# hello-robot/stretch_mujoco

Hardware: AMD Instinct MI355X
Metric: env-steps/sec (whole node), 4096 parallel Stretch envs in total (higher is better)
Workload: dtype f32

## Files before the change

stretch_mujoco_amd/csrc/smj_builds.h:

```cpp
#pragma once
#define SMJ_BUILDS_INCLUDED 1

#define SMJ_BUILDS(X) \
  X(step) X(pgs) X(prof) X(tall) X(mid) X(midp) X(big38) X(big38p) X(big50) X(big50p) X(big) X(sat) X(sat1) X(sat2) X(satp) X(sat32) X(sat32n)
#define SMJ_CARRIES_NEWTON 1
#define SMJ_CARRIES_PGS 2
#define SMJ_CARRIES_BOTH 3
#define SMJ_FAM_STD 0
#define SMJ_FAM_TALL 1
#define SMJ_FAM_MID 2
#define SMJ_FAM_BIG38 3
#define SMJ_FAM_BIG50 4
#define SMJ_FAM_BIG 5
#define SMJ_FAM_SAT16 6
#define SMJ_FAM_SAT32 7
#define SMJ_ROW_step    SMJ_FAM_STD,   SMJ_CARRIES_NEWTON, SMJ_CARRIES_NEWTON, 1, 0, 0
#define SMJ_ROW_pgs     SMJ_FAM_STD,   SMJ_CARRIES_PGS,    SMJ_CARRIES_PGS,    1, 0, 0
#define SMJ_ROW_prof    SMJ_FAM_STD,   SMJ_CARRIES_BOTH,   SMJ_CARRIES_BOTH,   1, 0, 1
#define SMJ_ROW_tall    SMJ_FAM_TALL,  SMJ_CARRIES_BOTH,   SMJ_CARRIES_BOTH,   1, 1, 0
#define SMJ_ROW_mid     SMJ_FAM_MID,   SMJ_CARRIES_NEWTON, SMJ_CARRIES_BOTH,   1, 0, 0
#define SMJ_ROW_midp    SMJ_FAM_MID,   SMJ_CARRIES_PGS,    SMJ_CARRIES_PGS,    1, 0, 0
#define SMJ_ROW_big38   SMJ_FAM_BIG38, SMJ_CARRIES_NEWTON, SMJ_CARRIES_BOTH,   1, 0, 0
#define SMJ_ROW_big38p  SMJ_FAM_BIG38, SMJ_CARRIES_PGS,    SMJ_CARRIES_PGS,    1, 0, 0
#define SMJ_ROW_big50   SMJ_FAM_BIG50, SMJ_CARRIES_NEWTON, SMJ_CARRIES_BOTH,   1, 0, 0
#define SMJ_ROW_big50p  SMJ_FAM_BIG50, SMJ_CARRIES_PGS,    SMJ_CARRIES_PGS,    1, 0, 0
#define SMJ_ROW_big     SMJ_FAM_BIG,   SMJ_CARRIES_BOTH,   SMJ_CARRIES_BOTH,   1, 1, 0
#define SMJ_ROW_sat     SMJ_FAM_SAT16, SMJ_CARRIES_NEWTON, SMJ_CARRIES_NEWTON, 1, 0, 0
#define SMJ_ROW_sat1    SMJ_FAM_SAT16, SMJ_CARRIES_PGS,    SMJ_CARRIES_PGS,    1, 0, 0
#define SMJ_ROW_sat2    SMJ_FAM_SAT16, SMJ_CARRIES_NEWTON, SMJ_CARRIES_NEWTON, 2, 0, 0
#define SMJ_ROW_satp    SMJ_FAM_SAT16, SMJ_CARRIES_PGS,    SMJ_CARRIES_PGS,    2, 0, 0
#define SMJ_ROW_sat32   SMJ_FAM_SAT32, SMJ_CARRIES_BOTH,   SMJ_CARRIES_BOTH,   1, 1, 0
#define SMJ_ROW_sat32n  SMJ_FAM_SAT32, SMJ_CARRIES_NEWTON, SMJ_CARRIES_NEWTON, 2, 1, 0
#define SMJ_LEAN_BUILDS(X) X(lean)
#define SMJ_ROW_lean    SMJ_FAM_STD,   SMJ_CARRIES_NEWTON, SMJ_CARRIES_NEWTON, 1, 0, 0
#define smj_step_kernel_step smj_step_kernel
#define smj_launch_step_step smj_launch_step

#define SMJ_CAT2(a, b) a##b
#define SMJ_CAT(a, b) SMJ_CAT2(a, b)
#define SMJ_STR2(a) #a
#define SMJ_STR(a) SMJ_STR2(a)
#define SMJ_COLUMN(m, ...) m(__VA_ARGS__, ~)
#define SMJ_COL0(a, ...) a
#define SMJ_COL1(a, b, ...) b
#define SMJ_COL2(a, b, c, ...) c
#define SMJ_COL3(a, b, c, d, ...) d
#define SMJ_COL4(a, b, c, d, e, ...) e
#define SMJ_COL5(a, b, c, d, e, f, ...) f
#ifdef SMJ_BUILD_TAG
// ... 94 lines not shown
  SmjLaunch launch;
  bool carries(int solver) const { return (solvers & (solver == 2 ? SMJ_CARRIES_NEWTON : SMJ_CARRIES_PGS)) != 0; }
};
#define SMJ_BUILD_DESC_INIT(launcher)                                                                                          \
  {SMJ_STR(SMJ_BUILD_TAG), SMJ_BUILD_FAMILY, SMJ_STR(SMJ_STEP_KERNEL), SMJ_BUILD_WORKER_NAME, {NVP, NBP, NENT, NEFC, NCON, NVS, NSAT}, \
   SMJ_DEBUG_FLOATS, SMJ_SOLVERS, SMJ_BUILD_WAVES, SMJ_PROFILING, launcher}
enum SmjBuildId {
#define X(tag) SMJ_B_##tag,
  SMJ_BUILDS(X)
#undef X
  SMJ_B_COUNT
};
#define X(tag) extern const SmjBuildDesc smj_build_##tag;
SMJ_BUILDS(X)
SMJ_LEAN_BUILDS(X)
#undef X
```

stretch_mujoco_amd/csrc/smj_capi.hip:

```cpp
#include <hip/hip_runtime.h>
#include <dlfcn.h>
#include <rccl/rccl.h>
#include <stdarg.h>
#include <sys/stat.h>
#include <time.h>
#include <unistd.h>
#include <stdio.h>
#include <stdlib.h>
#include <string.h>

#include <initializer_list>
#include <string>
#include <vector>

#include "../../include/smj.h"
#include "../../include/smj_build.h"
#include "smj_kernels.h"
#include "smj_step_plan.h"
#include "smj_model_load.h"
#include "smj_bvh.h"
#include "smj_meshlet.h"
#include "smj_render.h"
#include "smj_points.h"
#include "smj_hmap.h"
// ... 546 lines not shown
  StagePlan in, out;
  const SmjStageLayout& Y = c->layout;
  in.add(st.qpos, m.nq_all, Y.qpos); in.add(st.qvel, m.nv_all, Y.qvel); in.add(st.warm, m.nv_all, Y.warm);
  in.add(st.ctrl, m.nu, Y.ctrl); in.add(st.bctl, SMJ_BC_ROWS, Y.bctl); in.add(st.nstep, 1, Y.nstep);
  in.add(st.info, 4, Y.info);
  out = in;
  out.add(st.act_len, m.nu, Y.actlen); out.add(st.act_vel, m.nu, Y.actvel); out.add(st.base, 3, Y.base);
  if (read_flags & SMJ_READ_IMU) { out.add(st.gyro, 3, Y.gyro); out.add(st.accel, 3, Y.accel); }
  if (read_flags & SMJ_READ_POSES) out.add(st.xpose, 12 * m.nbody_all, Y.xpose);
  st.stage = c->stage;
  st.lay = Y;
  st.cost = c->cost;
  const SmjVariant& V = smj_variants[c->variant];
  const SmjCallFacts facts{c->num_envs, nsteps, st.debug != nullptr, st.prof != nullptr, c->has_esc};
  const SmjRoute route = smj_route_lean(smj_route(c->variant, c->model.solver, facts.prof_bound, c->opt.newton_two_waves, c->opt.pgs_two_waves, smj_builds),
                                        smj_lean_facts(c->model, st, c->opt.lean_build), smj_builds[SMJ_B_step], &smj_build_lean);
  const SmjStepPlan plan = smj_plan_step(V, route, c->opt, facts);
  c->last_primary = route.primary;
  if (plan.esc) {
#define X(name, field, type) c->model_esc.field = c->model.field;
    SMJ_SOLVER_OPTIONS(X)
#undef X
  }
  hipStream_t sm = (hipStream_t)stream;
  smj_launch_stage(in, c->stage, Y.stride, c->num_envs, st.ld, false, sm);
  st.progress = st.done_steps = st.sched = st.hot = nullptr;
  if (plan.clear_sched) {
    st.progress = c->progress;
    st.done_steps = c->progress + c->num_envs;
    st.sched = c->progress + 2 * (size_t)c->num_envs;
    st.hot = st.sched + SMJ_SCHED_WORDS;
// ... 394 lines not shown
```

stretch_mujoco_amd/csrc/smj_step_impl.h:

```cpp
#pragma once
#ifndef SMJ_PROFILING
#define SMJ_PROFILING 1
#endif
#include <cstddef>
#include "smj_model.h"
#include "smj_wave.h"
#include "smj_sat_mem.h"

#define JS (NVS + 1)
#define MS (NVS + 1)
#define SMJ_MINVAL 1e-15f
#define SMJ_MINIMP 0.0001f
#define SMJ_MAXIMP 0.9999f

enum { JT_FREE = 0, JT_BALL = 1, JT_SLIDE = 2, JT_HINGE = 3 };
enum { GT_PLANE = 0, GT_SPHERE = 2, GT_CAPSULE = 3, GT_ELLIPSOID = 4, GT_CYLINDER = 5, GT_BOX = 6, GT_MESH = 7 };
enum { CT_EQUALITY = 0, CT_FRICTION = 1, CT_LIMIT = 3, CT_CONTACT_FRICTIONLESS = 5, CT_CONTACT_ELLIPTIC = 7, CT_NONE = -1 };

#if NSAT > 0
#define NCGS (NCG + 1)
#define NSURV 128
#else
#define NCGS NCG
#endif
#if defined(SMJ_TWO_WAVES) && defined(SMJ_ONLY_NEWTON) && NSAT > 0 && !defined(SMJ_EMUL)
#define SMJ_SPLIT_COLLIDE 1
#else
#define SMJ_SPLIT_COLLIDE 0
#endif
#ifndef SMJ_W2_FORWARD
#define SMJ_W2_FORWARD SMJ_SPLIT_COLLIDE
#endif
#ifndef SMJ_W2_NEWTON
#define SMJ_W2_NEWTON SMJ_SPLIT_COLLIDE
#endif
#ifndef SMJ_W2_INTEGRATE
#define SMJ_W2_INTEGRATE SMJ_SPLIT_COLLIDE
#endif
struct TreeTmp {
  float cinert[NBP][10], crb[NBP][10], cvel[NBP][6], cfrc[NBP][6], buf[NVP][6], cdof[NVP][6], cdof_dot[NVP][6];
};

#define NEFP 64
#if NSAT > 0
#define NEFC_P SMJ_SAT_PGS
#else
#define NEFC_P (NEFC > 160 ? 160 : NEFC)
#endif
#define NPS ((NEFC_P + 63) / 64)
struct Smem {
  float MM[NVS][MS];
  float Mdiag[NVP], Dinv[NVP];
  float xpos[NBT][3], xquat[NBT][4], xmat[NBT][9], com[NBT][3];
  float xaxis[NVP][3], xanchor[NVP][3];
  float qpos[NVP + 8], qvel[NVP], ctrl[16], g[NVP], uu[NVP], w[NVP], qacc[NVP], warm[NVP], tmp[NVP];
  float act_force[16], act_len[16], act_vel[16], act_free[16];
  float bctl[SMJ_BC_ROWS];
  int etype[NEFC], eid[NEFC];
  int estate[NEFC];
  float epos[NEFC], emargin[NEFC], ediag[NEFC], efloss[NEFC], eR[NEFC], eK[NEFC], eBv[NEFC], eimp[NEFC], earef[NEFC],
      eb[NEFC], ef[NEFC];
  float cpos[NCON][3], cframe[NCON][9], cdist[NCON], cfric[NCON][5], csolref[NCON][2], csolimp[NCON][5], cmargin[NCON];
#if NSAT > 0
  int cdim[NCON], cefc[NCON];
  unsigned short cgeom1[NCON], cgeom2[NCON];
  int cpair[NCON];
#else
  int cdim[NCON], cgeom1[NCON], cgeom2[NCON], cefc[NCON];
#endif
#if NSAT > 0
  float J[NDR + 1][JS];
#else
  float J[NEFC][JS];
#endif
  union {
    TreeTmp t;
    struct {
      float pos[NCGS][3], mat[NCGS][9], cen[NCGS][3], half[NCGS][3];
      float ccen[NCGS][3], size[NCGS][3];
      int meta[NCGS];
      unsigned short list[1024];
// ... 28 lines not shown
#else
      union {
        float H[NVS][NVS + 1];
        float cH[NCON][36];
      };
#endif
      int rxi[3][NEFC > 64 ? NEFC - 64 : 1];
      float rxf[15][NEFC > 64 ? NEFC - 64 : 1];
    } n;
  } u;
#if NSAT > 0
  SatMem sat;
#endif
#if SMJ_SPLIT_COLLIDE
  int mbox[4];
#endif
  SMJ_DEV float* A(int cap) { return &J[cap][0]; }
};
#define ROWPASS(rb, ne) _Pragma("unroll") for (int rb = 0; rb < NEFC; rb += 64) if (rb == 0 || __builtin_expect((ne) > rb, 0))
#define ROWPASS_ALL(rb) _Pragma("unroll") for (int rb = 0; rb < NEFC; rb += 64)
#if NEFC > 128
#define ROWS_BEGIN_(rb, ne, LOAD) _Pragma("unroll") for (int rp_ = 0; rp_ < 2; rp_++) _Pragma("nounroll") for (int rb = rp_ ? 64 : 0; rp_ ? (rb < NEFC && (ne) > rb) : rb < 64; rb += 64) { NRow nrx_; if (rp_ && (LOAD)) rx_load(nrx_, rb); NRow& nr = rp_ ? nrx_ : nr0; (void)nr;
#define ROWS_END_RW(rb) if (rp_) rx_store(nrx_, rb); }
#else
#define ROWS_BEGIN_(rb, ne, LOAD) ROWPASS(rb, ne) { NRow nrx_; if (rb != 0 && (LOAD)) rx_load(nrx_, rb); NRow& nr = (rb != 0) ? nrx_ : nr0; (void)nr;
#define ROWS_END_RW(rb) if (rb != 0) rx_store(nrx_, rb); }
#endif
#define ROWS_BEGIN(rb, ne) ROWS_BEGIN_(rb, ne, true)
#define ROWS_END_RO() }
static inline int smj_pgs_rows_static() {
  const size_t a_sq = offsetof(Smem, J) + sizeof(float) * (NEFP * JS + NEFP * NEFP);
  if (a_sq > sizeof(Smem)) return 0;
  for (int n = NEFC_P & ~15; n > NEFP; n -= 16)
// ... 544 lines not shown
      }
    }
    SYNC();
    LANES {
      const int b = lane;
      if (b > 0 && b < nb) {
        const float* R = s.xmat[b];
        const float* I = bt.inl[lane];
        float Il[9] = {I[0], I[3], I[4], I[3], I[1], I[5], I[4], I[5], I[2]}, RI[9], T[9], Rt[9];
        mulmat3(RI, R, Il);
        for (int i = 0; i < 3; i++)
          for (int j = 0; j < 3; j++) Rt[3 * i + j] = R[3 * j + i];
        mulmat3(T, RI, Rt);
        float dif[3] = {xip[lane][0] - s.com[b][0], xip[lane][1] - s.com[b][1], xip[lane][2] - s.com[b][2]};
        const float mass = I[9], dd = dot3(dif, dif);
        float* c = s.u.t.cinert[b];
        c[0] = T[0] + mass * (dd - dif[0] * dif[0]); c[1] = T[4] + mass * (dd - dif[1] * dif[1]);
        c[2] = T[8] + mass * (dd - dif[2] * dif[2]); c[3] = T[1] - mass * dif[0] * dif[1];
        c[4] = T[2] - mass * dif[0] * dif[2]; c[5] = T[5] - mass * dif[1] * dif[2];
        c[6] = mass * dif[0]; c[7] = mass * dif[1]; c[8] = mass * dif[2]; c[9] = mass;
      }
      if (lane < nv) {
        const int d = lane, b = dt.body[lane];
        float off[3] = {s.com[b][0] - s.xanchor[d][0], s.com[b][1] - s.xanchor[d][1], s.com[b][2] - s.xanchor[d][2]};
        float* c = cdof[lane];
        const int jt = dt.jtype[lane], k = d - dt.first[lane];
        if (jt == JT_SLIDE || (jt == JT_FREE && k < 3)) {
          c[0] = c[1] = c[2] = 0;
          for (int x = 0; x < 3; x++) c[3 + x] = s.xaxis[d][x];
        } else {
          for (int x = 0; x < 3; x++) c[x] = s.xaxis[d][x];
          cross3(c + 3, s.xaxis[d], off);
        }
        for (int x = 0; x < 6; x++) s.u.t.cdof[d][x] = c[x];
        qvel_r[lane] = s.qvel[d];
      } else {
        for (int x = 0; x < 6; x++) cdof[lane][x] = 0;
        qvel_r[lane] = 0;
      }
    }
    SYNC();
    LANES {
      if (lane < nv)
        for (int x = 0; x < 6; x++) s.u.t.buf[lane][x] = cdof[lane][x] * qvel_r[lane];
    }
    SYNC();
    PL<float[6]> cvb;
    LANES {
      float sv[6] = {0, 0, 0, 0, 0, 0};
      if (lane > 0 && lane < nb) {
        const int da = bt.dofadr[lane], dn = bt.dofnum[lane];
#pragma unroll
        for (int u = 0; u < 6; u++) {
          const float on = u < dn ? 1.f : 0.f;
          const int a = da + (u < dn ? u : 0);
          for (int x = 0; x < 6; x++) sv[x] += on * s.u.t.buf[dn > 0 ? a : 0][x];
        }
      }
      for (int x = 0; x < 6; x++) { cvb[lane][x] = sv[x]; if (lane < NBP) s.u.t.cvel[lane][x] = sv[x]; }
    }
    SYNC();
#pragma unroll
    for (int r = 0; r < 6; r++) {
      if (r >= M.njump) break;
      PL<float[6]> up;
      PL<int> anc;
      LANES {
        const int a = bt.jump[lane][r];
        anc[lane] = a;
        for (int x = 0; x < 6; x++) up[lane][x] = s.u.t.cvel[a][x];
      }
      SYNC();
      LANES {
        if (anc[lane] > 0)
          for (int x = 0; x < 6; x++) { cvb[lane][x] += up[lane][x]; s.u.t.cvel[lane][x] = cvb[lane][x]; }
      }
      SYNC();
    }
    LANES {
      if (lane < nv) {
        const int b = dt.body[lane], pb = M.body_parentid[b], da = M.body_dofadr[b];
        float cv[6];
        for (int x = 0; x < 6; x++) cv[x] = s.u.t.cvel[pb][x];
        const uint64_t mk = dt.velmask[lane];
#pragma unroll
        for (int u = 0; u < 5; u++) {
          const int a = da + u;
          const float on = (a < lane && ((mk >> a) & 1)) ? 1.f : 0.f;
          for (int x = 0; x < 6; x++) cv[x] += on * s.u.t.buf[a < lane ? a : lane][x];
        }
        const int jt = dt.jtype[lane], k = lane - dt.first[lane];
        if (jt == JT_FREE && k < 3) { for (int x = 0; x < 6; x++) cdof_dot[lane][x] = 0; }
        else cross_motion(cdof_dot[lane], cv, cdof[lane]);
        for (int x = 0; x < 6; x++) s.u.t.cdof_dot[lane][x] = cdof_dot[lane][x];
      } else {
        for (int x = 0; x < 6; x++) cdof_dot[lane][x] = 0;
      }
    }
    {
      PL<float[10]> cr;
      LANES { for (int k = 0; k < 10; k++) cr[lane][k] = 0.f; }
      for (int x0 = 0; x0 < M.maxsubtree; x0 += 4) {
        LANES {
          if (lane > 0 && lane < nb) {
            const int sub = bt.subsize[lane];
#pragma unroll
            for (int u = 0; u < 4; u++) {
              const bool in = x0 + u < sub;
              const int x = lane + (in ? x0 + u : 0);
              const float on = in ? 1.f : 0.f;
              for (int k = 0; k < 10; k++) cr[lane][k] += on * s.u.t.cinert[x][k];
            }
          }
        }
      }
      LANES {
        if (lane < nb)
          for (int k = 0; k < 10; k++) s.u.t.crb[lane][k] = cr[lane][k];
      }
    }
    SYNC();
    LANES {
      if (lane < nv) {
        float bf[6];
        mul_inert_vec(bf, s.u.t.crb[dt.body[lane]], cdof[lane]);
        for (int x = 0; x < 6; x++) s.u.t.buf[lane][x] = bf[x];
      }
    }
    SYNC();
    LANES {
      for (int t = 0; t < NENT; t++) {
        const int i = et.i[lane][t], j = et.j[lane][t];
        if (i < 0) continue;
        float v = 0;
        for (int x = 0; x < 6; x++) v += s.u.t.cdof[j][x] * s.u.t.buf[i][x];
        if (i == j) { v += et.arm[lane][t]; s.Mdiag[i] = v; }
        s.MM[i][j] = v;
        if (i != j) s.MM[j][i] = v;
      }
    }
    SYNC();
  }

  SMJ_DEV void factor() {
    const int nv = M.nv;
    EntryTab et;
    load(et, false);
    for (int k = nv - 1; k >= 0; k--) {
      const float dkk = s.MM[k][k], dinv = 1.0f / dkk;
      LANES {
// ... 42 lines not shown
    BodyTab bt;
    load(bt);
    LANES {
      if (lane < 16) {
        float off[3] = {0, 0, 0}, F[3] = {0, 0, 0};
        int mlo = 0, mhi = 0;
        if (lane < M.ngc) {
          const int b = at.gc_body[lane];
          const float gm = at.gc_mass[lane];
          const float lp[3] = {at.gc_x[lane], at.gc_y[lane], at.gc_z[lane]};
          float pt[3];
          mulmat3vec(pt, s.xmat[b], lp);
          for (int k = 0; k < 3; k++) { off[k] = pt[k] + s.xpos[b][k] - s.com[b][k]; F[k] = -M.gravity[k] * gm; }
          mlo = at.gc_mlo[lane]; mhi = at.gc_mhi[lane];
        }
        float* o = s.u.t.buf[lane];
        for (int k = 0; k < 3; k++) { o[k] = off[k]; o[3 + k] = F[k]; }
        s.u.t.cfrc[lane][0] = __builtin_bit_cast(float, mlo); s.u.t.cfrc[lane][1] = __builtin_bit_cast(float, mhi);
      }
    }
    SYNC();
    LANES {
      if (lane < nv) {
        float acc = 0;
#pragma unroll
        for (int t = 0; t < 16; t++) {
          const uint64_t mk = mk64(__builtin_bit_cast(int, s.u.t.cfrc[t][0]), __builtin_bit_cast(int, s.u.t.cfrc[t][1]));
          const float* o = s.u.t.buf[t];
          float tv[3];
          cross3(tv, cdof[lane], o);
          const float v = (cdof[lane][3] + tv[0]) * o[3] + (cdof[lane][4] + tv[1]) * o[4] + (cdof[lane][5] + tv[2]) * o[5];
          acc += ((mk >> lane) & 1) ? v : 0.f;
        }
        frc_passive[lane] += acc;
      }
    }
    SYNC();
    LANES {
      if (lane < nv)
        for (int x = 0; x < 6; x++) s.u.t.buf[lane][x] = s.u.t.cdof_dot[lane][x] * s.qvel[lane];
    }
    SYNC();
    PL<float[6]> ca;
    LANES {
      float sv[6] = {0, 0, 0, 0, 0, 0};
      if (lane > 0 && lane < nb) {
        const int da = bt.dofadr[lane], dn = bt.dofnum[lane];
#pragma unroll
        for (int u = 0; u < 6; u++) {
          const float on = u < dn ? 1.f : 0.f;
          const int a = dn > 0 ? da + (u < dn ? u : 0) : 0;
          for (int x = 0; x < 6; x++) sv[x] += on * s.u.t.buf[a][x];
        }
      }
      for (int x = 0; x < 6; x++) { ca[lane][x] = sv[x]; if (lane < NBP) s.u.t.cfrc[lane][x] = sv[x]; }
    }
    SYNC();
#pragma unroll
    for (int r = 0; r < 6; r++) {
      if (r >= M.njump) break;
      PL<float[6]> up;
      PL<int> anc;
      LANES {
        const int a = bt.jump[lane][r];
        anc[lane] = a;
        for (int x = 0; x < 6; x++) up[lane][x] = s.u.t.cfrc[a][x];
      }
      SYNC();
      LANES {
        if (anc[lane] > 0)
          for (int x = 0; x < 6; x++) { ca[lane][x] += up[lane][x]; s.u.t.cfrc[lane][x] = ca[lane][x]; }
      }
      SYNC();
    }
    LANES {
      if (lane < nb) {
        const int b = lane;
        float t1[6] = {0, 0, 0, 0, 0, 0}, cf[6] = {0, 0, 0, 0, 0, 0};
        if (b > 0) {
          const float a[6] = {ca[lane][0], ca[lane][1], ca[lane][2], ca[lane][3] - M.gravity[0], ca[lane][4] - M.gravity[1], ca[lane][5] - M.gravity[2]};
          float t2[6];
          mul_inert_vec(t1, s.u.t.cinert[b], a);
          mul_inert_vec(t2, s.u.t.cinert[b], s.u.t.cvel[b]);
          cross_force(cf, s.u.t.cvel[b], t2);
        }
        for (int x = 0; x < 6; x++) s.u.t.cfrc[b][x] = t1[x] + cf[x];
      }
    }
    SYNC();
    {
      PL<float[6]> cfs;
      LANES { for (int k = 0; k < 6; k++) cfs[lane][k] = 0.f; }
      for (int x0 = 0; x0 < M.maxsubtree; x0 += 4) {
        LANES {
          if (lane < nv) {
            const int b = dt.body[lane], sub = dt.bsub[lane];
#pragma unroll
            for (int u = 0; u < 4; u++) {
              const bool in = x0 + u < sub;
              const int x = b + (in ? x0 + u : 0);
              const float on = in ? 1.f : 0.f;
              for (int k = 0; k < 6; k++) cfs[lane][k] += on * s.u.t.cfrc[x][k];
            }
          }
        }
      }
      LANES {
        float v = 0;
        if (lane < nv)
          for (int k = 0; k < 6; k++) v += cdof[lane][k] * cfs[lane][k];
        frc_bias[lane] = v;
      }
    }
    LANES {
      if (lane < nu) {
        const int a = lane;
        float len = 0, vel = 0;
// ... 1710 lines not shown
      while (mask) {
        const int l = ffs64(mask);
        mask &= mask - 1;
        const int t = wave_read(tt, l);
        const int* r = static_cast<const int*>(__builtin_assume_aligned(M.k_cprec + t * SMJ_CP_STRIDE, 16));
        const float sd[3] = {wave_read(sdx, l), wave_read(sdy, l), wave_read(sdz, l)};
        narrow_pair(r, uni(r[SMJ_CP_S1]), uni(r[SMJ_CP_S2]), sepbase ? sepbase + 4 * (t & (SMJ_SEP_SLOTS / 2 - 1)) : nullptr, t + 1,
                    sepbase && wave_read(stag, l) == t + 1, sd, pc, prof);
      }
      CTICK(SMJ_PROF_C_NARROW)
    }
    SYNC();
#undef CTICK
  }

  SMJ_DEV void make_constraint() {
    const int nv = M.nv, neq = M.neq, nfric = M.nfric, nlimit = M.nlimit;
    ROWPASS(rb, nefc) LANES {
      const int row = lane + rb;
      static_assert((64 * JS) % 4 == 0 && ((NEFC % 64) * JS) % 4 == 0, "row blocks are whole float4s");
      const int nrow = NEFC - rb < 64 ? NEFC - rb : 64, nf4 = nrow * JS / 4;
      Vec4* jz = reinterpret_cast<Vec4*>(&s.J[rb][0]);
      for (int k = lane; k < nf4; k += 64) jz[k] = Vec4{0.f, 0.f, 0.f, 0.f};
      if (row < NEFC) {
        s.etype[row] = CT_NONE; s.efloss[row] = 0; s.eid[row] = 0; s.epos[row] = 0; s.emargin[row] = 0; s.ediag[row] = 0;
      }
    }
    SYNC();
    int cap = newton() ? NEFC : M.pgs_cap > 0 ? M.pgs_cap : NEFC_P;
    if (M.row_limit > 0 && M.row_limit < cap) cap = M.row_limit;
// ... 44 lines not shown
    LANES {
      if (act[lane]) {
        const int r = row0 + popc64(lm & ((1ull << lane) - 1));
        if (r < cap) {
          const int side = lrow[1][lane];
          s.J[r][lrow[0][lane]] = (float)(-side);
          s.etype[r] = CT_LIMIT; s.eid[r] = lane;
          s.epos[r] = side * (asf(lrow[2][lane]) - lq[lane]);
          s.emargin[r] = asf(lrow[3][lane]); s.ediag[r] = asf(lrow[4][lane]);
        }
      }
    }
    row0 += popc64(lm);
    if (row0 > cap) { row0 = cap; flags |= SMJ_FLAG_EFC_OVERFLOW; }
    SYNC();
    PL<int> cact, cdimv, crow;
    PL<float> ctran, crot;
    LANES {
      int act = 0, dim = 0;
      float tran = 0, rot = 0;
      if (lane < ncon) {
        const int c = lane;
        dim = s.cdim[c];
        act = s.cdist[c] < s.cmargin[c];
        const int g1 = s.cgeom1[c], g2 = s.cgeom2[c], b1 = M.geom_bodyid[g1], b2 = M.geom_bodyid[g2];
        s.u.k.b1[c] = b1; s.u.k.b2[c] = b2;
        s.u.k.m1lo[c] = M.k_body_dofmask_lo[b1]; s.u.k.m1hi[c] = M.k_body_dofmask_hi[b1];
        s.u.k.m2lo[c] = M.k_body_dofmask_lo[b2]; s.u.k.m2hi[c] = M.k_body_dofmask_hi[b2];
        tran = M.geom_invweight0[2 * g1] + M.geom_invweight0[2 * g2];
        rot = M.geom_invweight0[2 * g1 + 1] + M.geom_invweight0[2 * g2 + 1];
// ... 1497 lines not shown
    sat_integrate(bad);
#endif
    if (wave_ballot(bad) != 0) {
      flags |= SMJ_FLAG_BAD_STATE;
      LANES {
        for (int k = lane; k < M.nq; k += 64) s.qpos[k] = M.qpos0[k];
        if (lane < nv) { s.qvel[lane] = 0.f; s.warm[lane] = 0.f; }
      }
#if NSAT > 0
      sat_reset_state();
#endif
      SYNC();
    }
  }

  SMJ_DEV void imu() {
    if (M.imu_site < 0 || (!S.gyro && !staged())) return;
    const int sid = M.imu_site, b = M.site_bodyid[sid];
    const uint64_t mk = mk64(M.k_body_dofmask_lo[b], M.k_body_dofmask_hi[b]);
    float cv[6], ca[6];
    for (int x = 0; x < 6; x++) {
      PL<float> tv, ta;
      LANES {
        const bool in = (mk >> lane) & 1;
        tv[lane] = in ? cdof[lane][x] * qvel_r[lane] : 0.f;
        ta[lane] = in ? cdof_dot[lane][x] * qvel_r[lane] + cdof[lane][x] * qacc_r[lane] : 0.f;
      }
      cv[x] = wave_sum(tv); ca[x] = wave_sum(ta);
    }
    for (int k = 0; k < 3; k++) ca[3 + k] -= M.gravity[k];
// ... 6 lines not shown
    cross3(t, cv, off);
    for (int k = 0; k < 3; k++) vlin[k] = cv[3 + k] + t[k];
    cross3(t, ca, off);
    for (int k = 0; k < 3; k++) alin[k] = ca[3 + k] + t[k];
    cross3(c2, cv, vlin);
    for (int k = 0; k < 3; k++) alin[k] += c2[k];
    mulmat3Tvec(gy, R, cv);
    mulmat3Tvec(ac, R, alin);
    if (staged()) {
      float* st = stage_row();
      LANES { if (lane < 3) { st[S.lay.gyro + lane] = gy[lane]; st[S.lay.accel + lane] = ac[lane]; } }
    } else {
      LANES { if (lane < 3) { S.gyro[lane * S.ld + env] = gy[lane]; S.accel[lane * S.ld + env] = ac[lane]; } }
    }
  }

  SMJ_DEV void dump_poses() {
    if (staged()) {
      float* st = stage_row() + S.lay.xpose;
      LANES {
        for (int k = lane; k < 12 * (M.nbody + M.nsat); k += 64) {
          const int b = k / 12, c = k - 12 * b;
          st[k] = c < 3 ? s.xpos[b][c] : s.xmat[b][c - 3];
        }
      }
      return;
    }
    if (!S.xpose) return;
    LANES {
      if (lane < M.nbody + M.nsat) {
// ... 82 lines not shown
#endif
  SMJ_DEV void run(int nsteps, unsigned read_flags) {
    const int want_imu = read_flags & 1;
    flags = 0; nefc = NEFC; ncon = 0; niter = 0;
    float pc[SMJ_PROF_SLOTS];
    for (int k = 0; k < SMJ_PROF_SLOTS; k++) pc[k] = 0.f;
    const bool prof = SMJ_PROFILING && S.prof != nullptr;
    const long long tlaunch = S.cost ? smj_clock() : 0;
    long long t0 = prof ? smj_clock() : 0, tstart = t0;
#define TICK(slot) if (prof) { const long long t1 = smj_clock(); pc[slot] += (float)(t1 - t0); t0 = t1; }
    setup();
    load_state();
    TICK(SMJ_PROF_SETUP)
    for (int st = 0; st < nsteps; st++) {
      const bool last = st == nsteps - 1;
#if SMJ_W2_FORWARD
      fork2(W2_SAT_FORWARD, env);
      kinematics();
      WG_BARRIER();
#else
      kinematics();
#if NSAT > 0
      sat_forward();
#endif
#endif
      if (last && (read_flags & 4)) dump_poses();
      TICK(SMJ_PROF_KIN)
      com_crb();
      if (last) dump_debug();
      TICK(SMJ_PROF_COMCRB)
// ... 17 lines not shown
          SYNC();
          ncon = ncon_planes;
          flags = flags_planes;
          serial_redo = true;
        }
        serial_redo = false;
      }
      if (last) dump_contacts();
      TICK(SMJ_PROF_COLLISION)
#if NSAT > 0
      make_constraint_sat(pc, prof);
#else
      if (!newton()) nefc = NEFC;
      make_constraint();
#endif
      TICK(SMJ_PROF_MAKECON)
      if (S.redo && !S.redo_worker && (flags & (SMJ_FLAG_EFC_OVERFLOW | SMJ_FLAG_CON_OVERFLOW))) {
        escalate(st);
        if (S.cost) { const int cst = (int)((smj_clock() - tlaunch) >> 6); LANES { if (lane == 0) st_coh(&S.cost[env], step_base ? ld_coh(&S.cost[env]) + cst : cst); } }
        return;
      }
#if NSAT > 0
      if (newton()) solve_newton(last, pc, t0, prof);
      else solve_pgs_sat(last, pc, t0, prof);
      if (last && debug_bound()) {
        LANES {
          if (lane >= 32 && lane - 32 < M.nsat)
            for (int k = 0; k < 6; k++) S.debug[(SMJ_DBG_SATQACC + 6 * (lane - 32) + k) * S.ld + env] = s.sat.x[SX_QA][lane - 32][k];
        }
      }
// ... 26 lines not shown
```

stretch_mujoco_amd/csrc/smj_step_tu.h:

```cpp
#pragma once
#ifdef SMJ_BUILDS_INCLUDED
#error "smj_step_tu.h must be the first include of its translation unit: smj_builds.h has to see SMJ_STEP_TU"
#endif
#define SMJ_STEP_TU 1
#include "smj_builds.h"
#include "smj_step_plan.h"
#include "smj_kernels.h"
#include "smj_step_impl.h"

#define SMJ_ALOAD(p) __hip_atomic_load((p), __ATOMIC_RELAXED, __HIP_MEMORY_SCOPE_AGENT)
#define SMJ_ASTORE(p, v) __hip_atomic_store((p), (v), __ATOMIC_RELAXED, __HIP_MEMORY_SCOPE_AGENT)
#define SMJ_WAIT_TICKS 300000000LL

struct SmjTicket { int env, steps, chunk; unsigned read_flags; bool go; };
static __device__ __forceinline__ SmjTicket smj_take_ticket(const DevState& S, int nsteps, unsigned read_flags) {
  SmjTicket t;
  int slot = blockIdx.x;
  t.chunk = 0; t.steps = nsteps; t.read_flags = read_flags; t.go = true; t.env = 0;
  if (S.pipe_len) {
    t.chunk = (int)blockIdx.x / S.B;
    slot = (int)blockIdx.x - t.chunk * S.B;
    const int base = t.chunk * S.pipe_len;
    t.steps = nsteps - base < S.pipe_len ? nsteps - base : S.pipe_len;
    if (base + t.steps < nsteps) t.read_flags = 0;
// ... 12 lines not shown
        break;
      }
      if (late) {
        if (threadIdx.x == 0) atomicOr(&reinterpret_cast<int*>(S.stage + (size_t)t.env * S.lay.stride)[S.lay.info + SMJ_INFO_FLAGS], SMJ_FLAG_PIPE_TIMEOUT);
        t.go = false;
        break;
      }
      __builtin_amdgcn_s_sleep(32);
    }
    coh_acquire();
  }
  return t;
}

#ifndef SMJ_KERNEL_ATTR
#define SMJ_KERNEL_ATTR
#endif
#ifdef SMJ_TWO_WAVES
#define SMJ_WG_THREADS 128
#else
#define SMJ_WG_THREADS 64
#endif
__global__ __launch_bounds__(SMJ_WG_THREADS) SMJ_KERNEL_ATTR void SMJ_STEP_KERNEL(const DevModel M, const DevState S, int nsteps, unsigned read_flags) {
  extern __shared__ __align__(16) unsigned char smj_lds[];
  Smem& smem = *reinterpret_cast<Smem*>(smj_lds);
#ifdef SMJ_TWO_WAVES
  if (threadIdx.x >= 64) {
#if SMJ_SPLIT_COLLIDE
    WG_BARRIER();
    if (uni(smem.mbox[0]) == StepKernel::W2_EXIT) return;
    StepKernel h(M, S, smem, uni(smem.mbox[1]));
    h.helper();
#else
    StepKernel h(M, S, smem, 0);
    h.pgs_helper();
#endif
    return;
  }
#endif
  const SmjTicket t = smj_take_ticket(S, nsteps, read_flags);
  if (t.go) {
    StepKernel k(M, S, smem, t.env);
    k.step_base = t.chunk * S.pipe_len;
    k.pipe_chunk = t.chunk;
    k.run(t.steps, t.read_flags);
    if (S.pipe_len && !k.parked) {
      coh_release();
      if (threadIdx.x == 0) SMJ_ASTORE(&S.progress[t.env], t.chunk + 1);
    }
  }
  if (S.sched && threadIdx.x == 0) atomicAdd(&S.sched[SMJ_SCHED_EXITED], 1);
#ifdef SMJ_TWO_WAVES
#if SMJ_SPLIT_COLLIDE
  if (threadIdx.x == 0) smem.mbox[0] = StepKernel::W2_EXIT;
#else
  if (threadIdx.x == 0) smem.sat.x[SX_MV][0][4] = __builtin_bit_cast(float, (int)StepKernel::PGS2_EXIT);
#endif
  WG_BARRIER();
#endif
}

#if defined(SMJ_WORKER_KERNEL)
static __device__ __forceinline__ void smj_worker_body(const DevModel& M, const DevState& S, Smem& smem, int nsteps, unsigned read_flags) {
  const int mode = S.redo_worker;
  long long t0 = mode == 2 ? wall_clock64() : 0;
  int exited_seen = -1;
  if (mode == 2) {
    if (S.pollers > 0 && *S.hot == 0) return;
// ... 112 lines not shown
```

stretch_mujoco_amd/csrc/smj_variants.h:

```cpp
#pragma once
#include "smj_builds.h"

enum { SMJ_NO_BUILD = -1, SMJ_NO_VARIANT = -1 };
enum SmjPipelines { SMJ_PIPE_NEVER = 0, SMJ_PIPE_ALWAYS, SMJ_PIPE_IF_BIG  };
struct SmjVariant {
  const char* name;
  int newton, pgs;
  int newton2, newton2_bit;
  int pgs2;
  int prof;
  int esc_variant, esc_build;
  SmjPipelines pipelines;
  int chunk_num, chunk_den;
  int poller_mult;
  bool escalates() const { return esc_variant != SMJ_NO_VARIANT || esc_build != SMJ_NO_BUILD; }
  int chunk_len(int pipeline) const { return (pipeline * chunk_num + chunk_den - 1) / chunk_den; }
};
#define B(tag) SMJ_B_##tag
#define NONE SMJ_NO_BUILD
static const SmjVariant smj_variants[7] = {
    {"standard", B(step),   B(pgs),    NONE,      0,  NONE,    B(prof), SMJ_NO_VARIANT, B(tall),  SMJ_PIPE_ALWAYS, 1, 1,  1},
    {"mid",      B(mid),    B(midp),   NONE,      0,  NONE,    NONE,    SMJ_NO_VARIANT, B(tall),  SMJ_PIPE_ALWAYS, 3, 2,  0},
    {"big38",    B(big38),  B(big38p), NONE,      0,  NONE,    NONE,    4,              NONE,     SMJ_PIPE_IF_BIG, 2, 1,  0},
    {"big50",    B(big50),  B(big50p), NONE,      0,  NONE,    NONE,    4,              NONE,     SMJ_PIPE_IF_BIG, 2, 1,  0},
// ... 30 lines not shown
struct SmjLeanFacts {
  int nroot;
  int manifold_cache;
  bool staged;
  bool debug_bound;
  bool prof_bound;
  int lean_build;
};
template <class Model, class State>
static inline SmjLeanFacts smj_lean_facts(const Model& m, const State& st, int lean_build) {
  return SmjLeanFacts{m.nroot, m.manifold_cache, st.stage != nullptr, st.debug != nullptr, st.prof != nullptr, lean_build};
}
static inline bool smj_lean_eligible(const SmjLeanFacts& f) {
  return f.lean_build != 0 && f.nroot == 1 && f.manifold_cache == 0 && f.staged && !f.debug_bound && !f.prof_bound;
}
static inline SmjRoute smj_route_lean(SmjRoute r, const SmjLeanFacts& f, const SmjBuildDesc* general, const SmjBuildDesc* lean) {
  if (lean && r.primary == general && smj_lean_eligible(f)) r.primary = lean;
  return r;
}
```

Measured before the change: 13.17 million.

## Run collision on a second wave in the lean build, overlapped with dynamics

The lean build becomes a two-wave kernel. A helper wave runs collision and convex collision while the main wave does com_crb, smooth forces and the start of constraint assembly, and the two meet through an LDS mailbox at a join inside make_constraint. To keep LDS within the standard family's budget, the tree temporaries are aliased onto the first rows of the J matrix rather than a separate union. The previous single-wave lean kernel is kept as lean2 and chosen when lean_build is 2. The IMU is recomputed with FP contraction turned off for the std family. The change doubles the waves per env and pins waves_per_eu to 2, which can cost occupancy and registers and adds barrier synchronisation.

```diff
diff --git a/stretch_mujoco_amd/csrc/smj_builds.h b/stretch_mujoco_amd/csrc/smj_builds.h
--- a/stretch_mujoco_amd/csrc/smj_builds.h
+++ b/stretch_mujoco_amd/csrc/smj_builds.h
@@ -32,7 +32,9 @@
 #define SMJ_ROW_sat32   SMJ_FAM_SAT32, SMJ_CARRIES_BOTH,   SMJ_CARRIES_BOTH,   1, 1, 0
 #define SMJ_ROW_sat32n  SMJ_FAM_SAT32, SMJ_CARRIES_NEWTON, SMJ_CARRIES_NEWTON, 2, 1, 0
 #define SMJ_LEAN_BUILDS(X) X(lean)
-#define SMJ_ROW_lean    SMJ_FAM_STD,   SMJ_CARRIES_NEWTON, SMJ_CARRIES_NEWTON, 1, 0, 0
+#define SMJ_ROW_lean    SMJ_FAM_STD,   SMJ_CARRIES_NEWTON, SMJ_CARRIES_NEWTON, 2, 0, 0
+#define SMJ_LEAN_TWIN_BUILDS(X) X(lean2)
+#define SMJ_ROW_lean2   SMJ_FAM_STD,   SMJ_CARRIES_NEWTON, SMJ_CARRIES_NEWTON, 1, 0, 0
 #define smj_step_kernel_step smj_step_kernel
 #define smj_launch_step_step smj_launch_step
 
@@ -157,4 +159,5 @@
 #define X(tag) extern const SmjBuildDesc smj_build_##tag;
 SMJ_BUILDS(X)
 SMJ_LEAN_BUILDS(X)
+SMJ_LEAN_TWIN_BUILDS(X)
 #undef X
diff --git a/stretch_mujoco_amd/csrc/smj_capi.hip b/stretch_mujoco_amd/csrc/smj_capi.hip
--- a/stretch_mujoco_amd/csrc/smj_capi.hip
+++ b/stretch_mujoco_amd/csrc/smj_capi.hip
@@ -584,7 +584,7 @@
   const SmjVariant& V = smj_variants[c->variant];
   const SmjCallFacts facts{c->num_envs, nsteps, st.debug != nullptr, st.prof != nullptr, c->has_esc};
   const SmjRoute route = smj_route_lean(smj_route(c->variant, c->model.solver, facts.prof_bound, c->opt.newton_two_waves, c->opt.pgs_two_waves, smj_builds),
-                                        smj_lean_facts(c->model, st, c->opt.lean_build), smj_builds[SMJ_B_step], &smj_build_lean);
+                                        smj_lean_facts(c->model, st, c->opt.lean_build), smj_builds[SMJ_B_step], smj_lean_pick(c->opt.lean_build, &smj_build_lean, &smj_build_lean2));
   const SmjStepPlan plan = smj_plan_step(V, route, c->opt, facts);
   c->last_primary = route.primary;
   if (plan.esc) {
diff --git a/stretch_mujoco_amd/csrc/smj_kernels_lean2.hip b/stretch_mujoco_amd/csrc/smj_kernels_lean2.hip
--- /dev/null
+++ b/stretch_mujoco_amd/csrc/smj_kernels_lean2.hip
@@ -0,0 +1,3 @@
+#define SMJ_BUILD_TAG lean2
+#define SMJ_LEAN 1
+#include "smj_step_tu.h"
diff --git a/stretch_mujoco_amd/csrc/smj_step_impl.h b/stretch_mujoco_amd/csrc/smj_step_impl.h
--- a/stretch_mujoco_amd/csrc/smj_step_impl.h
+++ b/stretch_mujoco_amd/csrc/smj_step_impl.h
@@ -36,6 +36,11 @@
 #endif
 #ifndef SMJ_W2_INTEGRATE
 #define SMJ_W2_INTEGRATE SMJ_SPLIT_COLLIDE
+#endif
+#if defined(SMJ_LEAN) && defined(SMJ_TWO_WAVES) && defined(SMJ_ONLY_NEWTON) && !(NSAT > 0) && !defined(SMJ_EMUL)
+#define SMJ_W2_COLLISION 1
+#else
+#define SMJ_W2_COLLISION 0
 #endif
 struct TreeTmp {
   float cinert[NBP][10], crb[NBP][10], cvel[NBP][6], cfrc[NBP][6], buf[NVP][6], cdof[NVP][6], cdof_dot[NVP][6];
@@ -65,6 +70,9 @@
   int cdim[NCON], cefc[NCON];
   unsigned short cgeom1[NCON], cgeom2[NCON];
   int cpair[NCON];
+#elif SMJ_W2_COLLISION
+  int cdim[NCON], cefc[NCON];
+  unsigned short cgeom1[NCON], cgeom2[NCON];
 #else
   int cdim[NCON], cgeom1[NCON], cgeom2[NCON], cefc[NCON];
 #endif
@@ -123,9 +131,20 @@
 #endif
 #if SMJ_SPLIT_COLLIDE
   int mbox[4];
+#elif SMJ_W2_COLLISION
+  int mbox[4];
 #endif
   SMJ_DEV float* A(int cap) { return &J[cap][0]; }
 };
+#if SMJ_W2_COLLISION
+#define SMJ_TT_ROWS 49
+static_assert(sizeof(TreeTmp) <= sizeof(float) * SMJ_TT_ROWS * JS && SMJ_TT_ROWS <= 64 && SMJ_TT_ROWS <= NEFC, "TreeTmp must fit the rows of J that every make_constraint() clears");
+static_assert(offsetof(Smem, J) % 16 == 0, "make_constraint() clears J with 16-byte stores");
+static_assert(sizeof(Smem) <= 40960, "the standard family's 32 LDS granules per env");
+#define SMJ_TT (*reinterpret_cast<TreeTmp*>(&s.J[0][0]))
+#else
+#define SMJ_TT s.u.t
+#endif
 #define ROWPASS(rb, ne) _Pragma("unroll") for (int rb = 0; rb < NEFC; rb += 64) if (rb == 0 || __builtin_expect((ne) > rb, 0))
 #define ROWPASS_ALL(rb) _Pragma("unroll") for (int rb = 0; rb < NEFC; rb += 64)
 #if NEFC > 128
@@ -700,7 +719,7 @@
         mulmat3(T, RI, Rt);
         float dif[3] = {xip[lane][0] - s.com[b][0], xip[lane][1] - s.com[b][1], xip[lane][2] - s.com[b][2]};
         const float mass = I[9], dd = dot3(dif, dif);
-        float* c = s.u.t.cinert[b];
+        float* c = SMJ_TT.cinert[b];
         c[0] = T[0] + mass * (dd - dif[0] * dif[0]); c[1] = T[4] + mass * (dd - dif[1] * dif[1]);
         c[2] = T[8] + mass * (dd - dif[2] * dif[2]); c[3] = T[1] - mass * dif[0] * dif[1];
         c[4] = T[2] - mass * dif[0] * dif[2]; c[5] = T[5] - mass * dif[1] * dif[2];
@@ -718,7 +737,7 @@
           for (int x = 0; x < 3; x++) c[x] = s.xaxis[d][x];
           cross3(c + 3, s.xaxis[d], off);
         }
-        for (int x = 0; x < 6; x++) s.u.t.cdof[d][x] = c[x];
+        for (int x = 0; x < 6; x++) SMJ_TT.cdof[d][x] = c[x];
         qvel_r[lane] = s.qvel[d];
       } else {
         for (int x = 0; x < 6; x++) cdof[lane][x] = 0;
@@ -728,7 +747,7 @@
     SYNC();
     LANES {
       if (lane < nv)
-        for (int x = 0; x < 6; x++) s.u.t.buf[lane][x] = cdof[lane][x] * qvel_r[lane];
+        for (int x = 0; x < 6; x++) SMJ_TT.buf[lane][x] = cdof[lane][x] * qvel_r[lane];
     }
     SYNC();
     PL<float[6]> cvb;
@@ -740,10 +759,10 @@
         for (int u = 0; u < 6; u++) {
           const float on = u < dn ? 1.f : 0.f;
           const int a = da + (u < dn ? u : 0);
-          for (int x = 0; x < 6; x++) sv[x] += on * s.u.t.buf[dn > 0 ? a : 0][x];
-        }
-      }
-      for (int x = 0; x < 6; x++) { cvb[lane][x] = sv[x]; if (lane < NBP) s.u.t.cvel[lane][x] = sv[x]; }
+          for (int x = 0; x < 6; x++) sv[x] += on * SMJ_TT.buf[dn > 0 ? a : 0][x];
+        }
+      }
+      for (int x = 0; x < 6; x++) { cvb[lane][x] = sv[x]; if (lane < NBP) SMJ_TT.cvel[lane][x] = sv[x]; }
     }
     SYNC();
 #pragma unroll
@@ -754,12 +773,12 @@
       LANES {
         const int a = bt.jump[lane][r];
         anc[lane] = a;
-        for (int x = 0; x < 6; x++) up[lane][x] = s.u.t.cvel[a][x];
+        for (int x = 0; x < 6; x++) up[lane][x] = SMJ_TT.cvel[a][x];
       }
       SYNC();
       LANES {
         if (anc[lane] > 0)
-          for (int x = 0; x < 6; x++) { cvb[lane][x] += up[lane][x]; s.u.t.cvel[lane][x] = cvb[lane][x]; }
+          for (int x = 0; x < 6; x++) { cvb[lane][x] += up[lane][x]; SMJ_TT.cvel[lane][x] = cvb[lane][x]; }
       }
       SYNC();
     }
@@ -767,18 +786,18 @@
       if (lane < nv) {
         const int b = dt.body[lane], pb = M.body_parentid[b], da = M.body_dofadr[b];
         float cv[6];
-        for (int x = 0; x < 6; x++) cv[x] = s.u.t.cvel[pb][x];
+        for (int x = 0; x < 6; x++) cv[x] = SMJ_TT.cvel[pb][x];
         const uint64_t mk = dt.velmask[lane];
 #pragma unroll
         for (int u = 0; u < 5; u++) {
           const int a = da + u;
           const float on = (a < lane && ((mk >> a) & 1)) ? 1.f : 0.f;
-          for (int x = 0; x < 6; x++) cv[x] += on * s.u.t.buf[a < lane ? a : lane][x];
+          for (int x = 0; x < 6; x++) cv[x] += on * SMJ_TT.buf[a < lane ? a : lane][x];
         }
         const int jt = dt.jtype[lane], k = lane - dt.first[lane];
         if (jt == JT_FREE && k < 3) { for (int x = 0; x < 6; x++) cdof_dot[lane][x] = 0; }
         else cross_motion(cdof_dot[lane], cv, cdof[lane]);
-        for (int x = 0; x < 6; x++) s.u.t.cdof_dot[lane][x] = cdof_dot[lane][x];
+        for (int x = 0; x < 6; x++) SMJ_TT.cdof_dot[lane][x] = cdof_dot[lane][x];
       } else {
         for (int x = 0; x < 6; x++) cdof_dot[lane][x] = 0;
       }
@@ -795,22 +814,22 @@
               const bool in = x0 + u < sub;
               const int x = lane + (in ? x0 + u : 0);
               const float on = in ? 1.f : 0.f;
-              for (int k = 0; k < 10; k++) cr[lane][k] += on * s.u.t.cinert[x][k];
+              for (int k = 0; k < 10; k++) cr[lane][k] += on * SMJ_TT.cinert[x][k];
             }
           }
         }
       }
       LANES {
         if (lane < nb)
-          for (int k = 0; k < 10; k++) s.u.t.crb[lane][k] = cr[lane][k];
+          for (int k = 0; k < 10; k++) SMJ_TT.crb[lane][k] = cr[lane][k];
       }
     }
     SYNC();
     LANES {
       if (lane < nv) {
         float bf[6];
-        mul_inert_vec(bf, s.u.t.crb[dt.body[lane]], cdof[lane]);
-        for (int x = 0; x < 6; x++) s.u.t.buf[lane][x] = bf[x];
+        mul_inert_vec(bf, SMJ_TT.crb[dt.body[lane]], cdof[lane]);
+        for (int x = 0; x < 6; x++) SMJ_TT.buf[lane][x] = bf[x];
       }
     }
     SYNC();
@@ -819,7 +838,7 @@
         const int i = et.i[lane][t], j = et.j[lane][t];
         if (i < 0) continue;
         float v = 0;
-        for (int x = 0; x < 6; x++) v += s.u.t.cdof[j][x] * s.u.t.buf[i][x];
+        for (int x = 0; x < 6; x++) v += SMJ_TT.cdof[j][x] * SMJ_TT.buf[i][x];
         if (i == j) { v += et.arm[lane][t]; s.Mdiag[i] = v; }
         s.MM[i][j] = v;
         if (i != j) s.MM[j][i] = v;
@@ -892,9 +911,9 @@
           for (int k = 0; k < 3; k++) { off[k] = pt[k] + s.xpos[b][k] - s.com[b][k]; F[k] = -M.gravity[k] * gm; }
           mlo = at.gc_mlo[lane]; mhi = at.gc_mhi[lane];
         }
-        float* o = s.u.t.buf[lane];
+        float* o = SMJ_TT.buf[lane];
         for (int k = 0; k < 3; k++) { o[k] = off[k]; o[3 + k] = F[k]; }
-        s.u.t.cfrc[lane][0] = __builtin_bit_cast(float, mlo); s.u.t.cfrc[lane][1] = __builtin_bit_cast(float, mhi);
+        SMJ_TT.cfrc[lane][0] = __builtin_bit_cast(float, mlo); SMJ_TT.cfrc[lane][1] = __builtin_bit_cast(float, mhi);
       }
     }
     SYNC();
@@ -903,8 +922,8 @@
         float acc = 0;
 #pragma unroll
         for (int t = 0; t < 16; t++) {
-          const uint64_t mk = mk64(__builtin_bit_cast(int, s.u.t.cfrc[t][0]), __builtin_bit_cast(int, s.u.t.cfrc[t][1]));
-          const float* o = s.u.t.buf[t];
+          const uint64_t mk = mk64(__builtin_bit_cast(int, SMJ_TT.cfrc[t][0]), __builtin_bit_cast(int, SMJ_TT.cfrc[t][1]));
+          const float* o = SMJ_TT.buf[t];
           float tv[3];
           cross3(tv, cdof[lane], o);
           const float v = (cdof[lane][3] + tv[0]) * o[3] + (cdof[lane][4] + tv[1]) * o[4] + (cdof[lane][5] + tv[2]) * o[5];
@@ -916,7 +935,7 @@
     SYNC();
     LANES {
       if (lane < nv)
-        for (int x = 0; x < 6; x++) s.u.t.buf[lane][x] = s.u.t.cdof_dot[lane][x] * s.qvel[lane];
+        for (int x = 0; x < 6; x++) SMJ_TT.buf[lane][x] = SMJ_TT.cdof_dot[lane][x] * s.qvel[lane];
     }
     SYNC();
     PL<float[6]> ca;
@@ -928,10 +947,10 @@
         for (int u = 0; u < 6; u++) {
           const float on = u < dn ? 1.f : 0.f;
           const int a = dn > 0 ? da + (u < dn ? u : 0) : 0;
-          for (int x = 0; x < 6; x++) sv[x] += on * s.u.t.buf[a][x];
-        }
-      }
-      for (int x = 0; x < 6; x++) { ca[lane][x] = sv[x]; if (lane < NBP) s.u.t.cfrc[lane][x] = sv[x]; }
+          for (int x = 0; x < 6; x++) sv[x] += on * SMJ_TT.buf[a][x];
+        }
+      }
+      for (int x = 0; x < 6; x++) { ca[lane][x] = sv[x]; if (lane < NBP) SMJ_TT.cfrc[lane][x] = sv[x]; }
     }
     SYNC();
 #pragma unroll
@@ -942,12 +961,12 @@
       LANES {
         const int a = bt.jump[lane][r];
         anc[lane] = a;
-        for (int x = 0; x < 6; x++) up[lane][x] = s.u.t.cfrc[a][x];
+        for (int x = 0; x < 6; x++) up[lane][x] = SMJ_TT.cfrc[a][x];
       }
       SYNC();
       LANES {
         if (anc[lane] > 0)
-          for (int x = 0; x < 6; x++) { ca[lane][x] += up[lane][x]; s.u.t.cfrc[lane][x] = ca[lane][x]; }
+          for (int x = 0; x < 6; x++) { ca[lane][x] += up[lane][x]; SMJ_TT.cfrc[lane][x] = ca[lane][x]; }
       }
       SYNC();
     }
@@ -958,11 +977,11 @@
         if (b > 0) {
           const float a[6] = {ca[lane][0], ca[lane][1], ca[lane][2], ca[lane][3] - M.gravity[0], ca[lane][4] - M.gravity[1], ca[lane][5] - M.gravity[2]};
           float t2[6];
-          mul_inert_vec(t1, s.u.t.cinert[b], a);
-          mul_inert_vec(t2, s.u.t.cinert[b], s.u.t.cvel[b]);
-          cross_force(cf, s.u.t.cvel[b], t2);
-        }
-        for (int x = 0; x < 6; x++) s.u.t.cfrc[b][x] = t1[x] + cf[x];
+          mul_inert_vec(t1, SMJ_TT.cinert[b], a);
+          mul_inert_vec(t2, SMJ_TT.cinert[b], SMJ_TT.cvel[b]);
+          cross_force(cf, SMJ_TT.cvel[b], t2);
+        }
+        for (int x = 0; x < 6; x++) SMJ_TT.cfrc[b][x] = t1[x] + cf[x];
       }
     }
     SYNC();
@@ -978,7 +997,7 @@
               const bool in = x0 + u < sub;
               const int x = b + (in ? x0 + u : 0);
               const float on = in ? 1.f : 0.f;
-              for (int k = 0; k < 6; k++) cfs[lane][k] += on * s.u.t.cfrc[x][k];
+              for (int k = 0; k < 6; k++) cfs[lane][k] += on * SMJ_TT.cfrc[x][k];
             }
           }
         }
@@ -2719,6 +2738,30 @@
 #undef CTICK
   }
 
+#if SMJ_W2_COLLISION
+  enum { W2_COLLIDE_ALL = 1, W2_EXIT = 2 };
+  SMJ_DEV void collide_helper() {
+    for (;;) {
+      flags = 0;
+      collision();
+      collision_convex(nullptr, false);
+      LANES { if (lane == 0) { s.mbox[2] = ncon; s.mbox[3] = flags; } }
+      WG_BARRIER();
+      WG_BARRIER();
+      if (uni(s.mbox[0]) == W2_EXIT) return;
+    }
+  }
+  SMJ_DEV void fork2(int cmd, int w1) {
+    LANES { if (lane == 0) { s.mbox[0] = cmd; s.mbox[1] = w1; } }
+    WG_BARRIER();
+  }
+  SMJ_DEV void join2() {
+    WG_BARRIER();
+    ncon = uni(s.mbox[2]);
+    flags |= uni(s.mbox[3]);
+  }
+#endif
+
   SMJ_DEV void make_constraint() {
     const int nv = M.nv, neq = M.neq, nfric = M.nfric, nlimit = M.nlimit;
     ROWPASS(rb, nefc) LANES {
@@ -2793,6 +2836,9 @@
     row0 += popc64(lm);
     if (row0 > cap) { row0 = cap; flags |= SMJ_FLAG_EFC_OVERFLOW; }
     SYNC();
+#if SMJ_W2_COLLISION
+    join2();
+#endif
     PL<int> cact, cdimv, crow;
     PL<float> ctran, crot;
     LANES {
@@ -4320,6 +4366,71 @@
     }
   }
 
+#if SMJ_BUILD_FAM == SMJ_FAM_STD
+#if defined(__clang__)
+#define SMJ_NO_CONTRACT _Pragma("clang fp contract(off)")
+#else
+#define SMJ_NO_CONTRACT
+#endif
+  SMJ_DEV static void imu_cross3(float* r, const float* a, const float* b) {
+    SMJ_NO_CONTRACT
+    const float p0 = a[1] * b[2], q0 = a[2] * b[1], p1 = a[2] * b[0], q1 = a[0] * b[2], p2 = a[0] * b[1], q2 = a[1] * b[0];
+    r[0] = p0 - q0; r[1] = p1 - q1; r[2] = p2 - q2;
+  }
+  SMJ_DEV static float imu_dot3(float a0, float a1, float a2, const float* v) {
+    SMJ_NO_CONTRACT
+    const float p0 = a0 * v[0], p1 = a1 * v[1], p2 = a2 * v[2];
+    const float s01 = p0 + p1;
+    return s01 + p2;
+  }
+  SMJ_DEV void imu() {
+    SMJ_NO_CONTRACT
+    if (M.imu_site < 0 || (!S.gyro && !staged())) return;
+    const int sid = M.imu_site, b = M.site_bodyid[sid];
+    const uint64_t mk = mk64(M.k_body_dofmask_lo[b], M.k_body_dofmask_hi[b]);
+    float cv[6], ca[6];
+    for (int x = 0; x < 6; x++) {
+      PL<float> tv, ta;
+      LANES {
+        const bool in = (mk >> lane) & 1;
+        const float pv = cdof[lane][x] * qvel_r[lane], pd = cdof_dot[lane][x] * qvel_r[lane], pa = cdof[lane][x] * qacc_r[lane];
+        tv[lane] = in ? pv : 0.f;
+        ta[lane] = in ? pd + pa : 0.f;
+      }
+      cv[x] = wave_sum(tv); ca[x] = wave_sum(ta);
+    }
+    for (int k = 0; k < 3; k++) ca[3 + k] -= M.gravity[k];
+    const float lp[3] = {M.site_pos[3 * sid], M.site_pos[3 * sid + 1], M.site_pos[3 * sid + 2]};
+    const float* X = s.xmat[b];
+    float sp[3], lm[9], R[9];
+    for (int i = 0; i < 3; i++) sp[i] = imu_dot3(X[3 * i], X[3 * i + 1], X[3 * i + 2], lp);
+    for (int k = 0; k < 9; k++) lm[k] = M.k_site_mat[9 * sid + k];
+    for (int i = 0; i < 3; i++)
+      for (int j = 0; j < 3; j++) {
+        const float col[3] = {lm[j], lm[3 + j], lm[6 + j]};
+        R[3 * i + j] = imu_dot3(X[3 * i], X[3 * i + 1], X[3 * i + 2], col);
+      }
+    float off[3];
+    for (int k = 0; k < 3; k++) { const float w = sp[k] + s.xpos[b][k]; off[k] = w - s.com[b][k]; }
+    float t[3], vlin[3], alin[3], c2[3], gy[3], ac[3];
+    imu_cross3(t, cv, off);
+    for (int k = 0; k < 3; k++) vlin[k] = cv[3 + k] + t[k];
+    imu_cross3(t, ca, off);
+    for (int k = 0; k < 3; k++) alin[k] = ca[3 + k] + t[k];
+    imu_cross3(c2, cv, vlin);
+    for (int k = 0; k < 3; k++) alin[k] += c2[k];
+    for (int j = 0; j < 3; j++) {
+      gy[j] = imu_dot3(R[j], R[3 + j], R[6 + j], cv);
+      ac[j] = imu_dot3(R[j], R[3 + j], R[6 + j], alin);
+    }
+    if (staged()) {
+      float* st = stage_row();
+      LANES { if (lane < 3) { st[S.lay.gyro + lane] = gy[lane]; st[S.lay.accel + lane] = ac[lane]; } }
+    } else {
+      LANES { if (lane < 3) { S.gyro[lane * S.ld + env] = gy[lane]; S.accel[lane * S.ld + env] = ac[lane]; } }
+    }
+  }
+#else
   SMJ_DEV void imu() {
     if (M.imu_site < 0 || (!S.gyro && !staged())) return;
     const int sid = M.imu_site, b = M.site_bodyid[sid];
@@ -4356,6 +4467,7 @@
       LANES { if (lane < 3) { S.gyro[lane * S.ld + env] = gy[lane]; S.accel[lane * S.ld + env] = ac[lane]; } }
     }
   }
+#endif
 
   SMJ_DEV void dump_poses() {
     if (staged()) {
@@ -4468,6 +4580,16 @@
     TICK(SMJ_PROF_SETUP)
     for (int st = 0; st < nsteps; st++) {
       const bool last = st == nsteps - 1;
+#if SMJ_W2_COLLISION
+      kinematics();
+      fork2(W2_COLLIDE_ALL, env);
+      if (last && (read_flags & 4)) dump_poses();
+      com_crb();
+      if (last) dump_debug();
+      smooth_forces(last);
+      make_constraint();
+      if (last) dump_contacts();
+#else
 #if SMJ_W2_FORWARD
       fork2(W2_SAT_FORWARD, env);
       kinematics();
@@ -4515,6 +4637,7 @@
       if (!newton()) nefc = NEFC;
       make_constraint();
 #endif
+#endif
       TICK(SMJ_PROF_MAKECON)
       if (S.redo && !S.redo_worker && (flags & (SMJ_FLAG_EFC_OVERFLOW | SMJ_FLAG_CON_OVERFLOW))) {
         escalate(st);
diff --git a/stretch_mujoco_amd/csrc/smj_step_tu.h b/stretch_mujoco_amd/csrc/smj_step_tu.h
--- a/stretch_mujoco_amd/csrc/smj_step_tu.h
+++ b/stretch_mujoco_amd/csrc/smj_step_tu.h
@@ -50,7 +50,11 @@
 }
 
 #ifndef SMJ_KERNEL_ATTR
+#if SMJ_W2_COLLISION
+#define SMJ_KERNEL_ATTR __attribute__((amdgpu_waves_per_eu(2, 2)))
+#else
 #define SMJ_KERNEL_ATTR
+#endif
 #endif
 #ifdef SMJ_TWO_WAVES
 #define SMJ_WG_THREADS 128
@@ -67,6 +71,11 @@
     if (uni(smem.mbox[0]) == StepKernel::W2_EXIT) return;
     StepKernel h(M, S, smem, uni(smem.mbox[1]));
     h.helper();
+#elif SMJ_W2_COLLISION
+    WG_BARRIER();
+    if (uni(smem.mbox[0]) == StepKernel::W2_EXIT) return;
+    StepKernel h(M, S, smem, uni(smem.mbox[1]));
+    h.collide_helper();
 #else
     StepKernel h(M, S, smem, 0);
     h.pgs_helper();
@@ -87,7 +96,7 @@
   }
   if (S.sched && threadIdx.x == 0) atomicAdd(&S.sched[SMJ_SCHED_EXITED], 1);
 #ifdef SMJ_TWO_WAVES
-#if SMJ_SPLIT_COLLIDE
+#if SMJ_SPLIT_COLLIDE || SMJ_W2_COLLISION
   if (threadIdx.x == 0) smem.mbox[0] = StepKernel::W2_EXIT;
 #else
   if (threadIdx.x == 0) smem.sat.x[SX_MV][0][4] = __builtin_bit_cast(float, (int)StepKernel::PGS2_EXIT);
diff --git a/stretch_mujoco_amd/csrc/smj_variants.h b/stretch_mujoco_amd/csrc/smj_variants.h
--- a/stretch_mujoco_amd/csrc/smj_variants.h
+++ b/stretch_mujoco_amd/csrc/smj_variants.h
@@ -68,6 +68,7 @@
 static inline bool smj_lean_eligible(const SmjLeanFacts& f) {
   return f.lean_build != 0 && f.nroot == 1 && f.manifold_cache == 0 && f.staged && !f.debug_bound && !f.prof_bound;
 }
+static inline const SmjBuildDesc* smj_lean_pick(int lean_build, const SmjBuildDesc* lean, const SmjBuildDesc* twin) { return lean_build == 2 && twin ? twin : lean; }
 static inline SmjRoute smj_route_lean(SmjRoute r, const SmjLeanFacts& f, const SmjBuildDesc* general, const SmjBuildDesc* lean) {
   if (lean && r.primary == general && smj_lean_eligible(f)) r.primary = lean;
   return r;
```

After: 13.97 million (median of 6 runs). +6.1%, better.
